# xvyaward/qeft

Measured on AMD Instinct MI355X. Metric: decode tokens/sec, Llama-2-7B w4 g128 r128, higher is better.
Workload: dtype f16; 1 GPU; llama-2-7b w4 g128 r128 full decode step, batch 1, greedy, KV context 69..1248 tokens (64-token context + 5 warm-up tokens before the timed region); layers=32, hipgraph=True, parallelism=single GPU

## Files before the change

include/qeft_hip.h:

```cpp
#ifndef QEFT_HIP_H
#define QEFT_HIP_H

#ifdef __cplusplus
extern "C" {
#endif

#define QEFT_OK 0
#define QEFT_ERR_BATCH 1
#define QEFT_ERR_SHAPE 2
#define QEFT_ERR_GROUP 3
#define QEFT_ERR_NULL 4
#define QEFT_ERR_LAUNCH 5
#define QEFT_ERR_ALIGN 6

typedef void* qeft_stream_t;

int qeft_abi_version(void);
const char* qeft_error_string(int code);
int qeft_last_hip_error(void);
const char* qeft_last_variant(void);

int qeft_gemv_w4(const void* x, const void* qweight, const void* scales, const void* scaled_zeros,
                 void* y, int m, int n, int k, int group_size, qeft_stream_t stream);

// ... 110 lines not shown
int qeft_token_begin_norm(const void* embed, const void* tok, const void* rope_tab, const int* pos, void* h32, void* rope_row,
                          const void* gamma, void* h_norm, float* ssq_out, int hidden, int vocab, int max_seq,
                          qeft_stream_t stream);
int qeft_rmsnorm_f32(const void* x32, const void* gamma, void* y, int m, int hidden, float eps, qeft_stream_t stream);
int qeft_rope_rows(void* x, const void* cos_tab, const void* sin_tab, int t, int n_heads, int row_stride,
                   qeft_stream_t stream);
int qeft_lm_head_f16(const void* h32, const void* gamma, const void* weight, void* logits, int hidden, int vocab, float eps,
                     qeft_stream_t stream);
int qeft_residual_norm(const void* h32, const void* add, const void* gamma, void* h32_out, void* h_norm, float* ssq_out,
                       int hidden, qeft_stream_t stream);

int qeft_gemm_w3_supported(int m, int n, int k, int group_size, int n_out);
int qeft_gemm_w3(const void* x, const void* qweight3, const void* scales, const void* scaled_zeros, const void* oweight,
                 const void* bias, void* y, int m, int n, int k, int group_size, int n_out, qeft_stream_t stream);
int qeft_gemm_w3_dx_supported(int m, int n, int k, int group_size, int n_out);
int qeft_gemm_w3_dx(const void* dy, const void* qweight3, const void* scales, const void* scaled_zeros, const void* oweight,
                    void* dx, int m, int n, int k, int group_size, int n_out, qeft_stream_t stream);

int qeft_gemv_w3(const void* x, const void* qweight3, const void* scales, const void* scaled_zeros,
                 const void* oweight_il, const void* bias, const void* residual, const void* sz_packed, void* y, int m,
                 int n, int k, int group_size, int n_out, qeft_stream_t stream);
int qeft_gemv_w3_group(const void* x, const void* norm_gamma, float norm_eps, int nparts,
                       const void* const* qweight3, const void* const* scales, const void* const* scaled_zeros,
                       const void* const* oweight_il, const void* const* bias, const void* const* sz_packed,
                       void* const* y, const int* n, int k, int group_size, int n_out, qeft_stream_t stream);
int qeft_gemv_w3_silu(const void* gate, const void* up, const void* qweight3, const void* scales,
                      const void* scaled_zeros, const void* oweight_il, const void* bias, const void* residual,
                      const void* sz_packed, void* y, int n, int k, int group_size, int n_out, qeft_stream_t stream);
int qeft_expand_w3(const void* qweight3, void* qweight4, int n, int k, int n_out, qeft_stream_t stream);

int qeft_token_begin(const void* embed, const void* tok, const void* rope_tab, const int* pos, void* h, void* rope_row,
                     int hidden, int vocab, int max_seq, qeft_stream_t stream);
int qeft_token_end(const void* logits, void* tok, int* pos, int vocab, int greedy, qeft_stream_t stream);

int qeft_decode_linear_m(const void* x, const void* qweight, const void* sz_packed, const void* oweight, const void* bias,
                         void* y, int n, int k, int group_size, int n_out, int mode, const void* residual,
                         const float* ssq_in, int n_ssq_in, float eps, const void* gamma_out, void* y_norm, float* ssq_out,
                         int m, qeft_stream_t stream);
long long qeft_gemv_v3_check_extents_m(int n, int k, int group_size, int n_out, int m, int mode, int n_ssq_in, int shrink_rows);
int qeft_token_begin_norm_m(const void* embed, const void* tokens, const void* rope_tab, const int* pos, void* h, void* rope_rows,
                            const void* gamma, void* h_norm, float* ssq_out, int hidden, int vocab, int max_seq, int m,
                            qeft_stream_t stream);
int qeft_attn_m_workspace_bytes(int n_heads, int n_split, int m);
int qeft_rope_attn_decode_m(const void* q, const void* k, const void* v, int qkv_stride, const void* cos_tab, const void* sin_tab,
                            int tab_stride, int tab_rows, void* k_cache, void* v_cache, const int* pos, const int* out_pos,
                            void* out, int out_stride, void* workspace, int n_split, int n_heads, int n_kv_heads, int max_seq,
                            int m, qeft_stream_t stream);
int qeft_lm_head_f16_m(const void* h32, const void* gamma, const void* weight, void* logits, int hidden, int vocab, float eps,
                       int m, qeft_stream_t stream);
int qeft_verify_greedy(const void* logits, const void* tokens, int m, int vocab, int greedy, void* out_tokens, int* n_accepted,
                       void* tok, int* pos, qeft_stream_t stream);

int qeft_token_begin_norm_batch(const void* embed, const void* tokens, const void* rope_tab, const int* slots, const int* pos, void* h,
                                void* rope_rows, const void* gamma, void* h_norm, float* ssq_out, int hidden, int vocab, int max_seq,
                                int n_slots, int m, qeft_stream_t stream);
int qeft_attn_batch_workspace_bytes(int n_heads, int n_split, int m);
int qeft_rope_attn_decode_batch(const void* q, const void* k, const void* v, int qkv_stride, const void* cos_tab, const void* sin_tab,
                                int tab_stride, int tab_rows, void* k_cache, void* v_cache, const int* slots, const int* pos,
                                const int* done, const int* out_pos, void* out, int out_stride, void* workspace, int n_split,
                                int n_slots, int n_heads, int n_kv_heads, int max_seq, int m, qeft_stream_t stream);
int qeft_token_end_batch(const void* logits, const int* slots, void* tokens, int* pos, const int* limit, const int* eos, int* done,
                         void* out, int* counter, int vocab, int out_cap, int n_slots, int m, qeft_stream_t stream);

int qeft_attn_kv8_workspace_bytes(int n_heads, int n_split, int m);
int qeft_rope_attn_decode_kv8(const void* q, const void* k, const void* v, int qkv_stride, const void* cos_tab, const void* sin_tab,
                              int tab_stride, int tab_rows, void* k_codes, void* v_codes, void* k_scales, void* v_scales,
// ... 107 lines not shown
```

qeft_amd/csrc/capi.hip:

```cpp
#include <hip/hip_runtime.h>

#include <cstdlib>
#include <cstring>
#include <stdint.h>

#include "../../include/qeft_hip.h"
#include "qeft_common.h"
#include "host_launch.h"
#include "gemm_w4.h"
#include "gemv_v3.h"
#include "decode_rows.h"
#include "decode_kv8.h"
#include "prefill_attn.h"
#include "attn_train.h"
#include "train_glue.h"

static thread_local int g_last_hip_error = 0;
thread_local const char* qeft::g_last_variant = "";
static bool small_m_route(int m, int n, bool have_workspace = false) {
    if (m <= 16) return true;
    if (have_workspace) return false;
    const int slices = (m + 15) / 16;
    return m <= 64 && (long long)slices * n <= 16384;
}
// ... 727 lines not shown
                          qeft_stream_t stream) {
    if (hidden < 8 || hidden % 8 != 0 || vocab < 1 || max_seq < 1) return QEFT_ERR_SHAPE;
    if (!embed || !tok || !h || !gamma || !h_norm || !ssq_out || (rope_row && (!rope_tab || !pos))) return QEFT_ERR_NULL;
    if (!aligned16(embed) || !aligned16(h) || !aligned16(gamma) || !aligned16(h_norm)) return QEFT_ERR_ALIGN;
    return finish(qeft::token_begin_norm_launch(embed, tok, rope_tab, pos, h, rope_row, gamma, h_norm, ssq_out, hidden, vocab,
                                                max_seq, (hipStream_t)stream));
}

int qeft_residual_norm(const void* h, const void* add, const void* gamma, void* h_out, void* h_norm, float* ssq_out,
                       int hidden, qeft_stream_t stream) {
    if (hidden < 8 || hidden % 8 != 0) return QEFT_ERR_SHAPE;
    if (!h || !h_out) return QEFT_ERR_NULL;
    if (gamma && (!h_norm || !ssq_out)) return QEFT_ERR_NULL;
    if (!aligned16(h) || !aligned16(h_out) || (add && !aligned16(add)) || (gamma && (!aligned16(gamma) || !aligned16(h_norm))))
        return QEFT_ERR_ALIGN;
    return finish(qeft::residual_norm_launch(h, add, gamma, h_out, h_norm, ssq_out, hidden, (hipStream_t)stream));
}

int qeft_token_begin(const void* embed, const void* tok, const void* rope_tab, const int* pos, void* h, void* rope_row,
                     int hidden, int vocab, int max_seq, qeft_stream_t stream) {
    if (hidden < 8 || hidden % 8 != 0 || vocab < 1 || max_seq < 1) return QEFT_ERR_SHAPE;
    if (!embed || !tok || !h || (rope_row && (!rope_tab || !pos))) return QEFT_ERR_NULL;
    if (!aligned16(embed) || !aligned16(h)) return QEFT_ERR_ALIGN;
    return finish(qeft::token_begin_launch(embed, tok, rope_tab, pos, h, rope_row, hidden, vocab, max_seq, (hipStream_t)stream));
}

int qeft_token_end(const void* logits, void* tok, int* pos, int vocab, int greedy, qeft_stream_t stream) {
    if (vocab < 1) return QEFT_ERR_SHAPE;
    if (!pos || (greedy && (!logits || !tok))) return QEFT_ERR_NULL;
    if (greedy && !aligned16(logits)) return QEFT_ERR_ALIGN;
    return finish(qeft::token_end_launch(logits, tok, pos, vocab, greedy, (hipStream_t)stream));
}

static bool verify_m_ok(int m) { return m >= 1 && m <= 8; }

int qeft_decode_linear_m(const void* x, const void* qweight, const void* sz_packed, const void* oweight, const void* bias,
                         void* y, int n, int k, int group_size, int n_out, int mode, const void* residual,
                         const float* ssq_in, int n_ssq_in, float eps, const void* gamma_out, void* y_norm, float* ssq_out,
                         int m, qeft_stream_t stream) {
    if (!verify_m_ok(m)) return QEFT_ERR_BATCH;
    if (m == 1)
        return qeft_decode_linear(x, qweight, sz_packed, oweight, bias, y, n, k, group_size, n_out, mode, residual, ssq_in, n_ssq_in,
                                  eps, gamma_out, y_norm, ssq_out, stream);
    if (int e = decode_linear_operands(x, qweight, 16, sz_packed, oweight, y, n_out)) return e;
    qeft::V3Args a;
    if (int e = v3_args(a, x, qweight, sz_packed, oweight, bias, y, n, k, group_size, n_out, mode)) return e;
    if (a.g.ngroups == 1 && k > 128) return QEFT_ERR_GROUP;
    if (int e = decode_linear_epilogue(a, mode, y, residual, ssq_in, n_ssq_in, eps, gamma_out, y_norm, ssq_out)) return e;
    a.m = m;
    hipError_t e = qeft::gemv_v3_multi_launch(a, mode, (hipStream_t)stream);
    if (e == hipErrorInvalidValue) return QEFT_ERR_SHAPE;
    return finish(e);
}

long long qeft_gemv_v3_check_extents_m(int n, int k, int group_size, int n_out, int m, int mode, int n_ssq_in, int shrink_rows) {
    qeft::V3Geom G{};
    if (!verify_m_ok(m) || v3_geom(G, n, k, group_size, n_out, mode) != QEFT_OK) return -1;
    if (G.ngroups == 1 && k > 128) return -1;
    if (n_ssq_in < 0 || n_ssq_in > qeft::V3_MAX_SSQ || shrink_rows < 0 || shrink_rows % 16 != 0 || shrink_rows >= n) return -1;
    return qeft::gemv_v3_count_out_of_range(G, n - shrink_rows, 0, false, 4) +
           qeft::gemv_v3_count_out_of_range_multi(G, n - shrink_rows, m, mode, n_ssq_in);
}

int qeft_token_begin_norm_m(const void* embed, const void* tokens, const void* rope_tab, const int* pos, void* h, void* rope_rows,
                            const void* gamma, void* h_norm, float* ssq_out, int hidden, int vocab, int max_seq, int m,
                            qeft_stream_t stream) {
// ... 597 lines not shown
```

qeft_amd/csrc/decode_aux.hip:

```cpp
#include <cstdlib>

#include "qeft_common.h"
#include "host_launch.h"
#include "decode_attn.h"

namespace qeft {

__device__ __forceinline__ float block_sum_256(float v, float* sm) {
    v = wave_sum(v);
    const int lane = threadIdx.x & 63, wave = threadIdx.x >> 6;
    __syncthreads();
    if (lane == 0) sm[wave] = v;
    __syncthreads();
    return sm[0] + sm[1] + sm[2] + sm[3];
}

__device__ __forceinline__ float block_max_256(float v, float* sm) {
#pragma unroll
    for (int o = 32; o > 0; o >>= 1) v = fmaxf(v, __shfl_xor(v, o));
    const int lane = threadIdx.x & 63, wave = threadIdx.x >> 6;
    __syncthreads();
    if (lane == 0) sm[wave] = v;
    __syncthreads();
    return fmaxf(fmaxf(sm[0], sm[1]), fmaxf(sm[2], sm[3]));
// ... 124 lines not shown
__global__ __launch_bounds__(256) void rmsnorm_f32_kernel(const float* __restrict__ x, const f16* __restrict__ gamma,
                                                          f16* __restrict__ y, int H, float eps) {
    __shared__ float sm[4];
    const size_t base = (size_t)blockIdx.x * H;
    float ss = 0.f;
    for (int i = threadIdx.x; i < H; i += 256) ss += x[base + i] * x[base + i];
    ss = block_sum_256(ss, sm);
    const float rs = rsqrtf(ss / (float)H + eps);
    for (int i = threadIdx.x; i < H; i += 256) y[base + i] = mul_f32_to_f16(x[base + i] * rs, (float)gamma[i]);
}

__global__ __launch_bounds__(256) void rope_rows_kernel(f16* __restrict__ x, const float* __restrict__ cs,
                                                        const float* __restrict__ sn, int H, int row_stride) {
    const int t = blockIdx.x, i = threadIdx.x & 63;
    const float c = cs[(size_t)t * 64 + i], s = sn[(size_t)t * 64 + i];
    for (int h = threadIdx.x >> 6; h < H; h += 4) {
        f16* p = x + (size_t)t * row_stride + h * 128;
        const float a = (float)p[i], b = (float)p[i + 64];
        p[i] = (f16)(a * c - b * s);
        p[i + 64] = (f16)(b * c + a * s);
    }
}

hipError_t rope_rows_launch(void* x, const void* cs, const void* sn, int T, int H, int row_stride, hipStream_t st) {
    hipLaunchKernelGGL(rope_rows_kernel, dim3(T), dim3(256), 0, st, (f16*)x, (const float*)cs, (const float*)sn, H, row_stride);
    return hipGetLastError();
}

template <int LPR>
__global__ __launch_bounds__(512) void lm_head_f16_kernel(const float* __restrict__ h32, const f16* __restrict__ gamma,
                                                          const f16* __restrict__ W, f16* __restrict__ logits, int vocab,
                                                          float eps, int rows_per_block) {
    constexpr int H = 512 * LPR;
    __shared__ float red[8];
    const int tid = threadIdx.x, lane = tid & 63;
    const int wave = __builtin_amdgcn_readfirstlane(tid >> 6);
    float xv[LPR][8];
    float ss = 0.f;
#pragma unroll
    for (int c = 0; c < LPR; ++c) {
        const f32x4 a = *(const f32x4*)(h32 + c * 512 + lane * 8), b = *(const f32x4*)(h32 + c * 512 + lane * 8 + 4);
#pragma unroll
        for (int j = 0; j < 4; ++j) {
            xv[c][j] = a[j];
            xv[c][4 + j] = b[j];
            ss += a[j] * a[j] + b[j] * b[j];
        }
    }
    ss = wave_sum(ss);
    const float rs = rsqrtf(ss / (float)H + eps);
    h2 xh[LPR][4];
#pragma unroll
    for (int c = 0; c < LPR; ++c) {
        const h8 g = *(const h8*)(gamma + c * 512 + lane * 8);
#pragma unroll
        for (int j = 0; j < 4; ++j)
            xh[c][j] = h2{mul_f32_to_f16(xv[c][2 * j] * rs, (float)g[2 * j]), mul_f32_to_f16(xv[c][2 * j + 1] * rs, (float)g[2 * j + 1])};
    }
    (void)red;
    const int r_end = min(vocab, (int)(blockIdx.x + 1) * rows_per_block);
    int r = blockIdx.x * rows_per_block + wave;
    u32x4 cur[LPR], nxt[LPR];
    auto load_row = [&](int row, u32x4 (&dst)[LPR]) {
        const u32x4* p = (const u32x4*)(W + (size_t)min(row, vocab - 1) * H) + lane;
#pragma unroll
        for (int c = 0; c < LPR; ++c) dst[c] = __builtin_nontemporal_load(p + c * 64);
    };
    load_row(r, cur);
    for (; r < r_end; r += 8) {
        load_row(r + 8, nxt);
        float acc = 0.f;
#pragma unroll
        for (int c = 0; c < LPR; ++c)
#pragma unroll
            for (int j = 0; j < 4; ++j) acc = __builtin_amdgcn_fdot2(as_h2(cur[c][j]), xh[c][j], acc, false);
        acc = wave_sum(acc);
        if (lane == 0) logits[r] = (f16)acc;
#pragma unroll
        for (int c = 0; c < LPR; ++c) cur[c] = nxt[c];
    }
}

hipError_t lm_head_f16_launch(const void* h32, const void* gamma, const void* W, void* logits, int H, int vocab, float eps,
                              hipStream_t st) {
    const int blocks = vocab >= 4096 ? 512 : (vocab + 7) / 8, rpb = (vocab + blocks - 1) / blocks;
    auto go = [&](auto kern) {
        hipLaunchKernelGGL(kern, dim3(blocks), dim3(512), 0, st, (const float*)h32, (const f16*)gamma, (const f16*)W, (f16*)logits,
                           vocab, eps, rpb);
        return hipGetLastError();
    };
    switch (H) {
        case 512: return go(lm_head_f16_kernel<1>);
        case 1024: return go(lm_head_f16_kernel<2>);
        case 2048: return go(lm_head_f16_kernel<4>);
        case 4096: return go(lm_head_f16_kernel<8>);
        case 5120: return go(lm_head_f16_kernel<10>);
        case 8192: return go(lm_head_f16_kernel<16>);
        default: return hipErrorInvalidValue;
    }
}

__global__ __launch_bounds__(1024) void token_end_kernel(const f16* __restrict__ logits, long long* __restrict__ tok,
                                                         int* __restrict__ pos, int vocab, int greedy) {
    __shared__ float bv[16];
    __shared__ int bi[16];
    const int t = threadIdx.x;
    if (greedy) {
        float best = -INFINITY;
        int idx = 0x7fffffff;
        for (int i = t * 8; i < vocab; i += 1024 * 8) {
            if (i + 8 <= vocab) {
                const h8 v = *(const h8*)(logits + i);
#pragma unroll
                for (int j = 0; j < 8; ++j)
                    if ((float)v[j] > best) { best = (float)v[j]; idx = i + j; }
            } else {
                for (int j = i; j < vocab; ++j)
                    if ((float)logits[j] > best) { best = (float)logits[j]; idx = j; }
            }
        }
#pragma unroll
        for (int o = 32; o > 0; o >>= 1) {
            const float ob = __shfl_xor(best, o);
            const int oi = __shfl_xor(idx, o);
            if (ob > best || (ob == best && oi < idx)) { best = ob; idx = oi; }
        }
        if ((t & 63) == 0) { bv[t >> 6] = best; bi[t >> 6] = idx; }
        __syncthreads();
        if (t == 0) {
            for (int w = 1; w < 16; ++w)
                if (bv[w] > best || (bv[w] == best && bi[w] < idx)) { best = bv[w]; idx = bi[w]; }
            *tok = idx == 0x7fffffff ? 0 : idx;
        }
    }
    if (t == 0) *pos = *pos + 1;
}

hipError_t token_begin_launch(const void* embed, const void* tok, const void* rope_tab, const int* pos, void* h,
                              void* rope_row, int hidden, int vocab, int max_seq, hipStream_t st) {
    hipLaunchKernelGGL(token_begin_kernel, dim3((hidden / 8 + 255) / 256), dim3(256), 0, st, (const f16*)embed,
                       (const long long*)tok, (const float*)rope_tab, pos, (f16*)h, (float*)rope_row, hidden, vocab, max_seq);
    return hipGetLastError();
}

int token_begin_norm_blocks(int hidden) { return (hidden / 8 + 255) / 256; }

hipError_t token_begin_norm_launch(const void* embed, const void* tok, const void* rope_tab, const int* pos, void* h,
                                   void* rope_row, const void* gamma, void* hnorm, float* ssq_out, int hidden, int vocab,
                                   int max_seq, hipStream_t st) {
    hipLaunchKernelGGL(token_begin_norm_kernel, dim3(token_begin_norm_blocks(hidden)), dim3(256), 0, st, (const f16*)embed,
                       (const long long*)tok, (const float*)rope_tab, pos, (float*)h, (float*)rope_row, (const f16*)gamma,
                       (f16*)hnorm, ssq_out, hidden, vocab, max_seq);
    return hipGetLastError();
}

hipError_t residual_norm_launch(const void* h, const void* add, const void* gamma, void* h_out, void* hnorm, float* ssq_out,
                                int hidden, hipStream_t st) {
    hipLaunchKernelGGL(residual_norm_kernel, dim3(token_begin_norm_blocks(hidden)), dim3(256), 0, st, (const float*)h,
                       (const f16*)add, (const f16*)gamma, (float*)h_out, (f16*)hnorm, ssq_out, hidden);
    return hipGetLastError();
}

hipError_t rmsnorm_f32_launch(const void* x, const void* gamma, void* y, int m, int H, float eps, hipStream_t st) {
    hipLaunchKernelGGL(rmsnorm_f32_kernel, dim3(m), dim3(256), 0, st, (const float*)x, (const f16*)gamma, (f16*)y, H, eps);
    return hipGetLastError();
}

hipError_t token_end_launch(const void* logits, void* tok, int* pos, int vocab, int greedy, hipStream_t st) {
    hipLaunchKernelGGL(token_end_kernel, dim3(1), dim3(1024), 0, st, (const f16*)logits, (long long*)tok, pos, vocab, greedy);
    return hipGetLastError();
}

hipError_t rmsnorm_launch(const void* x, const void* add, const void* gamma, void* res_out, void* y, int m, int H,
                          float eps, hipStream_t st) {
    hipLaunchKernelGGL(rmsnorm_kernel, dim3(m), dim3(256), 0, st, (const f16*)x, (const f16*)add, (const f16*)gamma,
                       (f16*)res_out, (f16*)y, H, eps);
    return hipGetLastError();
}

hipError_t silu_mul_launch(const void* gate, const void* up, void* out, int n, hipStream_t st) {
    hipLaunchKernelGGL(silu_mul_kernel, dim3((n / 8 + 255) / 256), dim3(256), 0, st, (const f16*)gate, (const f16*)up,
                       (f16*)out, n);
    return hipGetLastError();
}

unsigned long long* g_attn_dbg = nullptr;
#ifndef QEFT_ATTN_PRE1
#define QEFT_ATTN_PRE1 4
#endif
size_t attn_workspace_bytes(int n_heads, int S) { return S > 1 ? (attn_ctr_floats(n_heads) + (size_t)n_heads * S * kAttnRec) * 4 : 0; }

hipError_t rope_attn_decode_launch(const void* q, const void* k, const void* v, const void* cs, const void* sn, void* kc,
                                   void* vc, const int* pos, const int* out_pos, void* out, void* ws, int n_heads,
                                   int n_kv, int max_seq, int S, int tab_rows, hipStream_t st, bool k_ft_layout,
                                   const float* alibi_slopes) {
    const size_t smem = (size_t)(max_seq + 16) * 4 + 16 * 128 * 4 + 64 * 4 + 4 * 4 + 3 * 128 * 2;
    int dh = 1;
    auto launch = [&](auto kern) -> hipError_t {
        if (smem > 64 * 1024) {
            hipError_t e = hipFuncSetAttribute((const void*)kern, hipFuncAttributeMaxDynamicSharedMemorySize, (int)smem);
            if (e != hipSuccess) return e;
        }
// ... 133 lines not shown
```

qeft_amd/csrc/decode_verify.hip:

```cpp
#include "qeft_common.h"
#include "decode_attn.h"
#include "decode_rows.h"
#include "host_launch.h"

namespace qeft {

typedef float fx2 __attribute__((ext_vector_type(2)));

__global__ __launch_bounds__(256) void token_begin_norm_m_kernel(const f16* __restrict__ embed, const long long* __restrict__ toks,
                                                                 const float* __restrict__ rope_tab, const int* __restrict__ pos,
                                                                 float* __restrict__ h, float* __restrict__ rope_rows,
                                                                 const f16* __restrict__ gamma, f16* __restrict__ hnorm,
                                                                 float* __restrict__ ssq_out, int hidden, int vocab, int max_seq) {
    token_begin_norm_row(embed, toks, rope_tab, h, rope_rows, gamma, hnorm, ssq_out, hidden, vocab, max_seq,
                         [&](int row) { return *pos + row; });
}

hipError_t token_begin_norm_m_launch(const void* embed, const void* toks, const void* rope_tab, const int* pos, void* h,
                                     void* rope_rows, const void* gamma, void* hnorm, float* ssq_out, int hidden, int vocab,
                                     int max_seq, int m, hipStream_t st) {
    hipLaunchKernelGGL(token_begin_norm_m_kernel, dim3(token_begin_norm_blocks(hidden), m), dim3(256), 0, st, (const f16*)embed,
                       (const long long*)toks, (const float*)rope_tab, pos, (float*)h, (float*)rope_rows, (const f16*)gamma,
                       (f16*)hnorm, ssq_out, hidden, vocab, max_seq);
    return hipGetLastError();
// ... 248 lines not shown

size_t attn_m_workspace_bytes(int n_heads, int S, int m) { return S > 1 ? (attn_m_ctr_floats(n_heads) + (size_t)n_heads * m * S * kAttnRec) * 4 : 0; }

hipError_t rope_attn_m_launch(const AttnRowsArgs& a, hipStream_t st) {
    const int grp = a.n_heads / a.n_kv, hc = attn_m_chunk(grp, a.m), rows = hc * a.m;
    const int R = rows <= 8 ? 8 : rows <= 16 ? 16 : 32;
    const size_t smem = attn_m_smem_bytes(R);
    auto go = [&](auto kern) -> hipError_t {
        if (smem > 64 * 1024) {
            hipError_t e = hipFuncSetAttribute((const void*)kern, hipFuncAttributeMaxDynamicSharedMemorySize, (int)smem);
            if (e != hipSuccess) return e;
        }
        hipLaunchKernelGGL(kern, dim3(a.n_kv * (grp / hc) * a.S), dim3(256), smem, st, a.pos, a.out_pos, (const f16*)a.q, (const f16*)a.k,
                           (const f16*)a.v, (const float*)a.cs, (const float*)a.sn, (f16*)a.kc, (f16*)a.vc, (f16*)a.out, (float*)a.ws,
                           a.qkv_stride, a.out_stride, a.tab_stride, a.tab_rows, a.max_seq, a.n_heads, a.n_kv, a.S, a.m, hc);
        return hipGetLastError();
    };
    if (R == 8) return go(rope_attn_m_kernel<8>);
    if (R == 16) return go(rope_attn_m_kernel<16>);
    return go(rope_attn_m_kernel<32>);
}

template <int LPR>
__global__ __launch_bounds__(512) void lm_head_m_kernel(const float* __restrict__ h32, const f16* __restrict__ gamma,
                                                        const f16* __restrict__ W, f16* __restrict__ logits, int vocab, float eps,
                                                        int rows_per_block, int m) {
    constexpr int H = 512 * LPR;
    extern __shared__ __attribute__((aligned(16))) uint8_t smem_raw[];
    h8* const xs = (h8*)smem_raw;
    const int tid = threadIdx.x, lane = tid & 63;
    const int wave = __builtin_amdgcn_readfirstlane(tid >> 6);
    if (wave < m) {
        const float* hr = h32 + (size_t)wave * H;
        float xv[LPR][8];
        float ss = 0.f;
#pragma unroll
        for (int c = 0; c < LPR; ++c) {
            const f32x4 a = *(const f32x4*)(hr + c * 512 + lane * 8), b = *(const f32x4*)(hr + c * 512 + lane * 8 + 4);
#pragma unroll
            for (int j = 0; j < 4; ++j) {
                xv[c][j] = a[j];
                xv[c][4 + j] = b[j];
                ss += a[j] * a[j] + b[j] * b[j];
            }
        }
        ss = wave_sum(ss);
        const float rs = rsqrtf(ss / (float)H + eps);
#pragma unroll
        for (int c = 0; c < LPR; ++c) {
            const h8 g = *(const h8*)(gamma + c * 512 + lane * 8);
            h8 o;
#pragma unroll
            for (int j = 0; j < 8; ++j) o[j] = mul_f32_to_f16(xv[c][j] * rs, (float)g[j]);
            xs[((size_t)wave * LPR + c) * 64 + lane] = o;
        }
    }
    __syncthreads();
    const int r_end = min(vocab, (int)(blockIdx.x + 1) * rows_per_block);
    int r = blockIdx.x * rows_per_block + wave;
    u32x4 cur[LPR], nxt[LPR];
    auto load_row = [&](int row, u32x4 (&dst)[LPR]) {
        const u32x4* p = (const u32x4*)(W + (size_t)min(row, vocab - 1) * H) + lane;
#pragma unroll
        for (int c = 0; c < LPR; ++c) dst[c] = __builtin_nontemporal_load(p + c * 64);
    };
    load_row(r, cur);
    for (; r < r_end; r += 8) {
        load_row(r + 8, nxt);
        for (int i = 0; i < m; ++i) {
            float acc = 0.f;
#pragma unroll
            for (int c = 0; c < LPR; ++c) {
                const u32x4 xw = __builtin_bit_cast(u32x4, xs[((size_t)i * LPR + c) * 64 + lane]);
#pragma unroll
                for (int j = 0; j < 4; ++j) acc = __builtin_amdgcn_fdot2(as_h2(cur[c][j]), as_h2(xw[j]), acc, false);
            }
            acc = wave_sum(acc);
            if (lane == 0) logits[(size_t)i * vocab + r] = (f16)acc;
        }
#pragma unroll
        for (int c = 0; c < LPR; ++c) cur[c] = nxt[c];
    }
}

hipError_t lm_head_m_launch(const void* h32, const void* gamma, const void* W, void* logits, int H, int vocab, float eps, int m,
                            hipStream_t st) {
// ... 60 lines not shown
```

qeft_amd/csrc/host_launch.h:

```cpp
#pragma once
#include "qeft_common.h"

namespace qeft {

hipError_t token_begin_launch(const void* embed, const void* tok, const void* rope_tab, const int* pos, void* h,
                              void* rope_row, int hidden, int vocab, int max_seq, hipStream_t st);
int token_begin_norm_blocks(int hidden);
hipError_t token_begin_norm_launch(const void* embed, const void* tok, const void* rope_tab, const int* pos, void* h,
                                   void* rope_row, const void* gamma, void* hnorm, float* ssq_out, int hidden, int vocab,
                                   int max_seq, hipStream_t st);
hipError_t token_end_launch(const void* logits, void* tok, int* pos, int vocab, int greedy, hipStream_t st);
hipError_t residual_norm_launch(const void* h, const void* add, const void* gamma, void* h_out, void* hnorm, float* ssq_out,
                                int hidden, hipStream_t st);
hipError_t rmsnorm_launch(const void* x, const void* add, const void* gamma, void* res_out, void* y, int m, int H,
                          float eps, hipStream_t st);
hipError_t rmsnorm_f32_launch(const void* x, const void* gamma, void* y, int m, int H, float eps, hipStream_t st);
hipError_t rope_rows_launch(void* x, const void* cs, const void* sn, int T, int H, int row_stride, hipStream_t st);
hipError_t silu_mul_launch(const void* gate, const void* up, void* out, int n, hipStream_t st);
hipError_t lm_head_f16_launch(const void* h32, const void* gamma, const void* W, void* logits, int H, int vocab, float eps,
                              hipStream_t st);
size_t attn_workspace_bytes(int n_heads, int S);
hipError_t rope_attn_decode_launch(const void* q, const void* k, const void* v, const void* cs, const void* sn, void* kc,
                                   void* vc, const int* pos, const int* out_pos, void* out, void* ws, int n_heads,
                                   int n_kv, int max_seq, int S, int tab_rows, hipStream_t st, bool k_ft_layout = false,
                                   const float* alibi_slopes = nullptr);
hipError_t sqa_generic_launch(const void* q, const void* k, const void* v, void* kc, void* vc, const int* pos, const float* alibi,
                              void* out, int n_heads, int n_kv, int max_seq, int head_dim, hipStream_t st);
extern unsigned long long* g_attn_dbg;

hipError_t sample_launch(const void* logits, int vocab, int m, const int* params, const int* positions, void* tokens,
                         hipStream_t st);
hipError_t token_end_sample_launch(const void* logits, void* tok, int* pos, const int* params, int vocab, hipStream_t st);
hipError_t verify_sample_launch(const void* logits, const void* tokens, int m, int vocab, const int* params, int* work, void* out_tokens,
                                int* n_acc, void* tok, int* pos, hipStream_t st);
hipError_t token_end_sample_b_launch(const void* logits, const int* slot_tab, void* tok, int* pos_tab, const int* limit, const int* eos,
                                     int* done, void* out, int* ctr, const int* params, int vocab, int out_cap, int n_slots, int m,
                                     hipStream_t st);

hipError_t gemv_w4_dispatch(const GemvArgs& a, int m, hipStream_t st);
hipError_t gemv_w4_group_dispatch(GemvGroupArgs g, int nparts, hipStream_t st);
hipError_t gemv_w4_silu_dispatch(const GemvArgs& a, hipStream_t st);
hipError_t gemv_w4_smallm_dispatch(const GemvArgs& a, int m, hipStream_t st);
hipError_t gemv_w3_dispatch(const GemvArgs& a, int m, hipStream_t st);
hipError_t gemv_w3_group_dispatch(GemvGroupArgs g, int nparts, hipStream_t st);
// ... 24 lines not shown
```

qeft_amd/llama.py:

```python
import ctypes
import os
import math
import types
from dataclasses import dataclass

import torch
import torch.nn as nn

from . import _lib, fuse, qeft_cuda
from .qlinear import QuantLinear
from .quant import fake_quantize, minmax_params


@dataclass
class LlamaShape:
    hidden: int
    inter: int
    n_layers: int
    n_heads: int
    n_kv_heads: int
    vocab: int
    max_seq: int = 512
    rms_eps: float = 1e-5
    rope_theta: float = 10000.0
# ... 910 lines not shown
        self._head(h32, self.hn, self.logits, None, st)
        self._token_end(st)

    def _lin_m(self, b, m, st):
        s, lib = self.m.shape, self.lib
        g, no, eps = s.group_size, s.n_out, s.rms_eps
        xn, ssq = b.xn.data_ptr(), b.ssq.data_ptr()

        def lin(op, x, y, mode=0, residual=None, ssq_in=None, n_ssq=0, gamma_out=None):
            return lib.qeft_decode_linear_m(x, op.qweight.data_ptr(), op.sz_packed.data_ptr(), op.oweight.data_ptr() if no else None,
                                            None, y, op.outfeatures, op.infeatures, g, no, mode, residual, ssq_in, n_ssq, eps,
                                            gamma_out, xn if gamma_out else None, ssq if gamma_out else None, m, st)
        return lin

    def _v3_layers(self, b, lin, attn, only=None):
        ck, layers = _lib.check, self.m.model.layers
        xn, ssq, h32 = b.xn.data_ptr(), b.ssq.data_ptr(), b.h32.data_ptr()
        qkv, att, act = b.qkv.data_ptr(), b.att.data_ptr(), b.act.data_ptr()

        lin_qkv, lin_o, lin_gu, lin_d = (lin if only in (None, tag) else (lambda *a, **kw: 0) for tag in ("qkv", "o", "gu", "d"))
        n_ssq = self.n_ssq_tb
        for li, L in enumerate(layers):
            pk = self.v3ops[li]
            ck(lin_qkv(pk["qkv"], xn, qkv, ssq_in=ssq, n_ssq=n_ssq))
            if attn is not None:
                attn(li)
            ck(lin_o(pk["o"], att, h32, residual=h32, gamma_out=L.post_attention_layernorm.weight.data_ptr()))
            n_ssq = self.n_ssq_lin
            ck(lin_gu(pk["gu"], xn, act, mode=1, ssq_in=ssq, n_ssq=n_ssq))
            nxt = layers[li + 1].input_layernorm.weight.data_ptr() if li + 1 < len(layers) else None
            ck(lin_d(pk["d"], act, h32, residual=h32, gamma_out=nxt))

    @torch.no_grad()
    def _launch_token_v3(self, linears_only=False, only=None):
        s, lib, ck, b = self.m.shape, self.lib, _lib.check, self.row1
        st = torch.cuda.current_stream(self.dev).cuda_stream
        g, no, eps = s.group_size, s.n_out, s.rms_eps
        xn, ssq, h32 = b.xn.data_ptr(), b.ssq.data_ptr(), b.h32.data_ptr()
        entry = lib.qeft_decode_linear_w3 if self.bits == 3 else lib.qeft_decode_linear

        def lin(op, x, y, mode=0, residual=None, ssq_in=None, n_ssq=0, gamma_out=None):
            return entry(x, op.qweight.data_ptr(), op.sz_packed.data_ptr(), op.oweight.data_ptr() if no else None, None, y,
                         op.outfeatures, op.infeatures, g, no, mode, residual, ssq_in, n_ssq, eps, gamma_out,
                         xn if gamma_out else None, ssq if gamma_out else None, st)
        if linears_only:
            return self._v3_layers(b, lin, None, only)
        ck(lib.qeft_token_begin_norm(self.m.model.embed_tokens.weight.data_ptr(), self.tok.data_ptr(), self.rope_tab.data_ptr(),
                                     self.pos.data_ptr(), h32, self.rope_row.data_ptr(),
                                     self.m.model.layers[0].input_layernorm.weight.data_ptr(), xn, ssq, s.hidden, s.vocab,
                                     s.max_seq, st))
        q, k, v = self.q.data_ptr(), self.k.data_ptr(), self.v.data_ptr()
        self._v3_layers(b, lin, lambda li: self._attn(li, q, k, v, self.att_pos[li], self.att, st), only)
        self._token_tail(h32, st)

    @torch.no_grad()
    def _launch_token_tp3(self, linears_only=False, only=None):
        s, lib, ck = self.m.shape, self.lib, _lib.check
        st = torch.cuda.current_stream(self.dev).cuda_stream
        g, no, eps = s.group_size, s.n_out, s.rms_eps
        layers = self.m.model.layers
        cur, oth = self.h32, self.part32
        zero = self.zero32.data_ptr()

        def hnorm(op, h, gamma, y, mode=0):
            return lib.qeft_decode_linear_hnorm(h.data_ptr(), gamma.data_ptr(), op.qweight.data_ptr(), op.sz_packed.data_ptr(),
                                                op.oweight.data_ptr() if no else None, None, y, op.outfeatures, op.infeatures, g,
                                                no, mode, eps, st)

        def partial(op, x, h, y):
            return lib.qeft_decode_linear(x, op.qweight.data_ptr(), op.sz_packed.data_ptr(), op.oweight.data_ptr() if no else None,
                                          None, y.data_ptr(), op.outfeatures, op.infeatures, g, no, 0,
                                          h.data_ptr() if self.rank == 0 else zero, None, 0, eps, None, None, None, st)

        def pick(tag, fn):
            return fn if only in (None, tag) else (lambda *a, **kw: 0)
        if not linears_only:
            ck(lib.qeft_token_begin_norm(self.m.model.embed_tokens.weight.data_ptr(), self.tok.data_ptr(),
                                         self.rope_tab.data_ptr(), self.pos.data_ptr(), cur.data_ptr(), self.rope_row.data_ptr(),
                                         layers[0].input_layernorm.weight.data_ptr(), self.xn.data_ptr(), self.ssq.data_ptr(), s.hidden,
                                         s.vocab, s.max_seq, st))
        qp = self.qkv_loc.data_ptr()
        for li, L in enumerate(layers):
            pk = self.tp3ops[li]
            ck(pick("qkv", hnorm)(pk["qkv"], cur, L.input_layernorm.weight, qp))
            if not linears_only:
                self._attn(li, qp, qp + self.hs * 2, qp + (self.hs + self.kvs) * 2, pk["att_pos"], pk["x_o"], st)
# ... 46 lines not shown
        self.sample_rec.copy_(torch.tensor(params.record(), dtype=torch.int32))
        self.sampling = params

    def step(self):
        if self.host_pos >= self.m.shape.max_seq:
            raise RuntimeError(f"KV cache full: position {self.host_pos} >= max_seq {self.m.shape.max_seq}")
        self._check_fresh()
        sp = self._split_for(self.host_pos)
        if self.use_graph:
            g = self.graphs.get(self._step_key(sp))
            if g is None:
                g = self.capture(split=sp)
            g.replay()
        else:
            self.attn_split = sp
            self._launch_token()
        self.host_pos += 1

    MULTI = int(os.environ.get("QEFT_MULTI_TOKENS", "8"))

    def run(self, n_tokens):
        assert self.greedy or self.sampling is not None, \
            "run() feeds every token's successor to the next: greedy or sampled decoding only"
        self._check_fresh()
        multi_ok = self.use_graph and os.environ.get("QEFT_MULTI_TOKEN_GRAPH") != "0"
        while n_tokens > 0:
            p, m = self.host_pos, self.MULTI
            sp = self._split_for(p)
            if multi_ok and n_tokens >= m and p + m <= self.m.shape.max_seq and self._split_for(p + m - 1) == sp:
                key = (sp, "sample", m) if self.sampling is not None else (sp, True, m)
                g = self.graphs.get(key)
                if g is None:
                    self.attn_split = sp
                    g = self.graphs[key] = capture_graph(self.dev, self._launch_token, m, (self.pos, self.tok))
                g.replay()
                self.host_pos += m
                n_tokens -= m
            else:
                self.step()
                n_tokens -= 1

    VERIFY_MAX = 8

    def _m_row_unsupported(self):
        if self.tp or self.tp3:
            return "the verify pass runs on the single-GPU engine only (this engine is tensor-parallel)"
        if self.bits != 4:
            return f"the verify pass runs on 4-bit weights only (this engine has {self.bits}-bit weights)"
        if not self.v3:
            return "the verify pass runs on the v3 engine only (QEFT_ENGINE_V2=1, or shapes the v3 GEMV does not take)"
        return None

    def _verify_unsupported(self):
        why = self._m_row_unsupported()
        if why is None and self.kv_dtype != "fp16" and not getattr(self, "kv8_verify", False):
            return (f'the verify pass runs on an fp16 KV cache only (this engine has kv_dtype="{self.kv_dtype}"; '
                    f'build it with kv8_verify=True for the verify pass over an fp8 KV cache)')
        return why

    def _verify_bufs(self):
        vb = getattr(self, "_vb", None)
        if vb is not None:
            return vb
        s, dev, M = self.m.shape, self.dev, self.VERIFY_MAX
        ws_bytes = self.lib.qeft_attn_m_kv8_workspace_bytes if self.kv_dtype == "fp8" else self.lib.qeft_attn_m_workspace_bytes
        vb = m_row_buffers(self, M, ws_bytes(s.n_heads, 8, M))
        vb.toks = torch.zeros(M, dtype=torch.long, device=dev)
# ... 96 lines not shown
```

Measured before the change: 756.7 tokens/s.

## Fuse greedy argmax with next token's embed/norm/rope into one turn kernel

```diff
diff --git a/include/qeft_hip.h b/include/qeft_hip.h
--- a/include/qeft_hip.h
+++ b/include/qeft_hip.h
@@ -166,6 +166,8 @@
 int qeft_token_begin(const void* embed, const void* tok, const void* rope_tab, const int* pos, void* h, void* rope_row,
                      int hidden, int vocab, int max_seq, qeft_stream_t stream);
 int qeft_token_end(const void* logits, void* tok, int* pos, int vocab, int greedy, qeft_stream_t stream);
+int qeft_token_turn(const void* logits, void* tok, int* pos, const void* embed, const void* rope_tab, void* h32, void* rope_row,
+                    const void* gamma, void* h_norm, float* ssq_out, int hidden, int vocab, int max_seq, qeft_stream_t stream);
 
 int qeft_decode_linear_m(const void* x, const void* qweight, const void* sz_packed, const void* oweight, const void* bias,
                          void* y, int n, int k, int group_size, int n_out, int mode, const void* residual,
diff --git a/qeft_amd/csrc/capi.hip b/qeft_amd/csrc/capi.hip
--- a/qeft_amd/csrc/capi.hip
+++ b/qeft_amd/csrc/capi.hip
@@ -783,6 +783,15 @@
     return finish(qeft::token_end_launch(logits, tok, pos, vocab, greedy, (hipStream_t)stream));
 }
 
+int qeft_token_turn(const void* logits, void* tok, int* pos, const void* embed, const void* rope_tab, void* h, void* rope_row,
+                    const void* gamma, void* h_norm, float* ssq_out, int hidden, int vocab, int max_seq, qeft_stream_t stream) {
+    if (hidden < 8 || hidden % 8 != 0 || hidden > 8192 || vocab < 1 || max_seq < 1) return QEFT_ERR_SHAPE;
+    if (!logits || !tok || !pos || !embed || !rope_tab || !h || !rope_row || !gamma || !h_norm || !ssq_out) return QEFT_ERR_NULL;
+    if (!aligned16(logits) || !aligned16(embed) || !aligned16(h) || !aligned16(gamma) || !aligned16(h_norm)) return QEFT_ERR_ALIGN;
+    return finish(qeft::token_turn_launch(logits, tok, pos, embed, rope_tab, h, rope_row, gamma, h_norm, ssq_out, hidden, vocab,
+                                          max_seq, (hipStream_t)stream));
+}
+
 static bool verify_m_ok(int m) { return m >= 1 && m <= 8; }
 
 int qeft_decode_linear_m(const void* x, const void* qweight, const void* sz_packed, const void* oweight, const void* bias,
diff --git a/qeft_amd/csrc/decode_aux.hip b/qeft_amd/csrc/decode_aux.hip
--- a/qeft_amd/csrc/decode_aux.hip
+++ b/qeft_amd/csrc/decode_aux.hip
@@ -180,43 +180,56 @@
                                                           const f16* __restrict__ W, f16* __restrict__ logits, int vocab,
                                                           float eps, int rows_per_block) {
     constexpr int H = 512 * LPR;
-    __shared__ float red[8];
+    constexpr int CUR0 = LPR == 16 ? 0 : LPR == 8 ? 4 : LPR;
+    constexpr int XH0 = LPR == 8 ? 2 : LPR;
     const int tid = threadIdx.x, lane = tid & 63;
     const int wave = __builtin_amdgcn_readfirstlane(tid >> 6);
-    float xv[LPR][8];
+    const int r_end = min(vocab, (int)(blockIdx.x + 1) * rows_per_block);
+    int r = blockIdx.x * rows_per_block + wave;
+    if (r >= r_end) return;
+    u32x4 cur[LPR], nxt[LPR];
+    auto load_row = [&](int row, u32x4 (&dst)[LPR], int c0, int c1) {
+        const u32x4* p = (const u32x4*)(W + (size_t)min(row, vocab - 1) * H) + lane;
+#pragma unroll
+        for (int c = c0; c < c1; ++c) dst[c] = __builtin_nontemporal_load(p + c * 64);
+    };
+    f32x4 xa[LPR], xb[LPR];
+    h8 g[LPR];
+#pragma unroll
+    for (int c = 0; c < LPR; ++c) {
+        xa[c] = *(const f32x4*)(h32 + c * 512 + lane * 8);
+        xb[c] = *(const f32x4*)(h32 + c * 512 + lane * 8 + 4);
+    }
+#pragma unroll
+    for (int c = 0; c < LPR; ++c) g[c] = *(const h8*)(gamma + c * 512 + lane * 8);
+    load_row(r, cur, 0, CUR0);
+    __builtin_amdgcn_sched_barrier(0);
     float ss = 0.f;
 #pragma unroll
-    for (int c = 0; c < LPR; ++c) {
-        const f32x4 a = *(const f32x4*)(h32 + c * 512 + lane * 8), b = *(const f32x4*)(h32 + c * 512 + lane * 8 + 4);
-#pragma unroll
-        for (int j = 0; j < 4; ++j) {
-            xv[c][j] = a[j];
-            xv[c][4 + j] = b[j];
-            ss += a[j] * a[j] + b[j] * b[j];
-        }
-    }
+    for (int c = 0; c < LPR; ++c)
+#pragma unroll
+        for (int j = 0; j < 4; ++j) ss += xa[c][j] * xa[c][j] + xb[c][j] * xb[c][j];
     ss = wave_sum(ss);
     const float rs = rsqrtf(ss / (float)H + eps);
     h2 xh[LPR][4];
-#pragma unroll
-    for (int c = 0; c < LPR; ++c) {
-        const h8 g = *(const h8*)(gamma + c * 512 + lane * 8);
-#pragma unroll
-        for (int j = 0; j < 4; ++j)
-            xh[c][j] = h2{mul_f32_to_f16(xv[c][2 * j] * rs, (float)g[2 * j]), mul_f32_to_f16(xv[c][2 * j + 1] * rs, (float)g[2 * j + 1])};
-    }
-    (void)red;
-    const int r_end = min(vocab, (int)(blockIdx.x + 1) * rows_per_block);
-    int r = blockIdx.x * rows_per_block + wave;
-    u32x4 cur[LPR], nxt[LPR];
-    auto load_row = [&](int row, u32x4 (&dst)[LPR]) {
-        const u32x4* p = (const u32x4*)(W + (size_t)min(row, vocab - 1) * H) + lane;
-#pragma unroll
-        for (int c = 0; c < LPR; ++c) dst[c] = __builtin_nontemporal_load(p + c * 64);
+    auto norm_chunk = [&](int c) {
+#pragma unroll
+        for (int j = 0; j < 2; ++j) {
+            xh[c][j] = h2{mul_f32_to_f16(xa[c][2 * j] * rs, (float)g[c][2 * j]), mul_f32_to_f16(xa[c][2 * j + 1] * rs, (float)g[c][2 * j + 1])};
+            xh[c][2 + j] = h2{mul_f32_to_f16(xb[c][2 * j] * rs, (float)g[c][4 + 2 * j]), mul_f32_to_f16(xb[c][2 * j + 1] * rs, (float)g[c][4 + 2 * j + 1])};
+        }
     };
-    load_row(r, cur);
-    for (; r < r_end; r += 8) {
-        load_row(r + 8, nxt);
+#pragma unroll
+    for (int c = 0; c < XH0; ++c) norm_chunk(c);
+    if constexpr (CUR0 < LPR) {
+        __builtin_amdgcn_sched_barrier(0);
+        load_row(r, cur, CUR0, LPR);
+        __builtin_amdgcn_sched_barrier(0);
+    }
+#pragma unroll
+    for (int c = XH0; c < LPR; ++c) norm_chunk(c);
+    do {
+        load_row(r + 8, nxt, 0, LPR);
         float acc = 0.f;
 #pragma unroll
         for (int c = 0; c < LPR; ++c)
@@ -226,7 +239,8 @@
         if (lane == 0) logits[r] = (f16)acc;
 #pragma unroll
         for (int c = 0; c < LPR; ++c) cur[c] = nxt[c];
-    }
+        r += 8;
+    } while (r < r_end);
 }
 
 hipError_t lm_head_f16_launch(const void* h32, const void* gamma, const void* W, void* logits, int H, int vocab, float eps,
@@ -248,40 +262,116 @@
     }
 }
 
+__device__ __forceinline__ int greedy_argmax_1024(const f16* __restrict__ logits, int vocab, float* bv, int* bi) {
+    constexpr int kPass = 1024 * 8, kPre = 4;
+    const int t = threadIdx.x;
+    float best = -INFINITY;
+    int idx = 0x7fffffff;
+    auto tail = [&](int i) {
+        for (int j = i; j < vocab; ++j)
+            if ((float)logits[j] > best) { best = (float)logits[j]; idx = j; }
+    };
+    if (vocab <= kPre * kPass) {
+        h8 v[kPre] = {};
+        if (vocab >= 8) {
+            const int last = (vocab & ~7) - 8;
+#pragma unroll
+            for (int p = 0; p < kPre; ++p) v[p] = *(const h8*)(logits + min(t * 8 + p * kPass, last));
+        }
+        __builtin_amdgcn_sched_barrier(0);
+#pragma unroll
+        for (int p = 0; p < kPre; ++p) {
+            const int i = t * 8 + p * kPass;
+            if (i + 8 <= vocab) {
+#pragma unroll
+                for (int j = 0; j < 8; ++j)
+                    if ((float)v[p][j] > best) { best = (float)v[p][j]; idx = i + j; }
+            } else if (i < vocab) {
+                tail(i);
+            }
+        }
+    } else {
+        for (int i = t * 8; i < vocab; i += kPass) {
+            if (i + 8 <= vocab) {
+                const h8 v = *(const h8*)(logits + i);
+#pragma unroll
+                for (int j = 0; j < 8; ++j)
+                    if ((float)v[j] > best) { best = (float)v[j]; idx = i + j; }
+            } else {
+                tail(i);
+            }
+        }
+    }
+#pragma unroll
+    for (int o = 32; o > 0; o >>= 1) {
+        const float ob = __shfl_xor(best, o);
+        const int oi = __shfl_xor(idx, o);
+        if (ob > best || (ob == best && oi < idx)) { best = ob; idx = oi; }
+    }
+    if ((t & 63) == 0) { bv[t >> 6] = best; bi[t >> 6] = idx; }
+    __syncthreads();
+    if (t == 0)
+        for (int w = 1; w < 16; ++w)
+            if (bv[w] > best || (bv[w] == best && bi[w] < idx)) { best = bv[w]; idx = bi[w]; }
+    return idx == 0x7fffffff ? 0 : idx;
+}
+
 __global__ __launch_bounds__(1024) void token_end_kernel(const f16* __restrict__ logits, long long* __restrict__ tok,
                                                          int* __restrict__ pos, int vocab, int greedy) {
     __shared__ float bv[16];
     __shared__ int bi[16];
     const int t = threadIdx.x;
     if (greedy) {
-        float best = -INFINITY;
-        int idx = 0x7fffffff;
-        for (int i = t * 8; i < vocab; i += 1024 * 8) {
-            if (i + 8 <= vocab) {
-                const h8 v = *(const h8*)(logits + i);
-#pragma unroll
-                for (int j = 0; j < 8; ++j)
-                    if ((float)v[j] > best) { best = (float)v[j]; idx = i + j; }
-            } else {
-                for (int j = i; j < vocab; ++j)
-                    if ((float)logits[j] > best) { best = (float)logits[j]; idx = j; }
-            }
-        }
-#pragma unroll
-        for (int o = 32; o > 0; o >>= 1) {
-            const float ob = __shfl_xor(best, o);
-            const int oi = __shfl_xor(idx, o);
-            if (ob > best || (ob == best && oi < idx)) { best = ob; idx = oi; }
-        }
-        if ((t & 63) == 0) { bv[t >> 6] = best; bi[t >> 6] = idx; }
-        __syncthreads();
-        if (t == 0) {
-            for (int w = 1; w < 16; ++w)
-                if (bv[w] > best || (bv[w] == best && bi[w] < idx)) { best = bv[w]; idx = bi[w]; }
-            *tok = idx == 0x7fffffff ? 0 : idx;
-        }
+        const int idx = greedy_argmax_1024(logits, vocab, bv, bi);
+        if (t == 0) *tok = idx;
     }
     if (t == 0) *pos = *pos + 1;
+}
+
+__global__ __launch_bounds__(1024) void token_turn_kernel(const f16* __restrict__ logits, long long* __restrict__ tok,
+                                                          int* __restrict__ pos, const f16* __restrict__ embed,
+                                                          const float* __restrict__ rope_tab, float* __restrict__ h,
+                                                          float* __restrict__ rope_row, const f16* __restrict__ gamma,
+                                                          f16* __restrict__ hnorm, float* __restrict__ ssq_out, int hidden,
+                                                          int vocab, int max_seq) {
+    __shared__ float bv[16];
+    __shared__ int bi[16];
+    __shared__ float sm[16];
+    __shared__ int tok_s;
+    const int t = threadIdx.x, i = t * 8;
+    const int p1 = *pos + 1;
+    const bool mine = i < hidden, rope = t >= 896 && rope_row;
+    const h8 g = *(const h8*)(gamma + (mine ? i : 0));
+    const float rv = rope_tab[(size_t)min(max(p1, 0), max_seq - 1) * 128 + (rope ? t - 896 : 0)];
+    __builtin_amdgcn_sched_barrier(0);
+    const int idx = greedy_argmax_1024(logits, vocab, bv, bi);
+    if (t == 0) {
+        *tok = idx;
+        *pos = p1;
+        tok_s = idx;
+    }
+    __syncthreads();
+    const int tk = min(max(tok_s, 0), vocab - 1);
+    float ss = 0.f;
+    if (mine) {
+        const h8 v = *(const h8*)(embed + (size_t)tk * hidden + i);
+        h8 o;
+#pragma unroll
+        for (int j = 0; j < 8; ++j) {
+            ss += (float)v[j] * (float)v[j];
+            o[j] = mul_f32_to_f16((float)v[j], (float)g[j]);
+            h[i + j] = (float)v[j];
+        }
+        *(h8*)(hnorm + i) = o;
+    }
+    ss = wave_sum(ss);
+    if ((t & 63) == 0) sm[t >> 6] = ss;
+    __syncthreads();
+    if ((t & 255) == 0 && t * 8 < hidden) {
+        const int w = t >> 6;
+        ssq_out[t >> 8] = sm[w] + sm[w + 1] + sm[w + 2] + sm[w + 3];
+    }
+    if (rope) rope_row[t - 896] = rv;
 }
 
 hipError_t token_begin_launch(const void* embed, const void* tok, const void* rope_tab, const int* pos, void* h,
@@ -316,6 +406,15 @@
 
 hipError_t token_end_launch(const void* logits, void* tok, int* pos, int vocab, int greedy, hipStream_t st) {
     hipLaunchKernelGGL(token_end_kernel, dim3(1), dim3(1024), 0, st, (const f16*)logits, (long long*)tok, pos, vocab, greedy);
+    return hipGetLastError();
+}
+
+hipError_t token_turn_launch(const void* logits, void* tok, int* pos, const void* embed, const void* rope_tab, void* h,
+                             void* rope_row, const void* gamma, void* hnorm, float* ssq_out, int hidden, int vocab, int max_seq,
+                             hipStream_t st) {
+    hipLaunchKernelGGL(token_turn_kernel, dim3(1), dim3(1024), 0, st, (const f16*)logits, (long long*)tok, pos, (const f16*)embed,
+                       (const float*)rope_tab, (float*)h, (float*)rope_row, (const f16*)gamma, (f16*)hnorm, ssq_out, hidden, vocab,
+                       max_seq);
     return hipGetLastError();
 }
 
diff --git a/qeft_amd/csrc/decode_verify.hip b/qeft_amd/csrc/decode_verify.hip
--- a/qeft_amd/csrc/decode_verify.hip
+++ b/qeft_amd/csrc/decode_verify.hip
@@ -304,26 +304,31 @@
     const int wave = __builtin_amdgcn_readfirstlane(tid >> 6);
     if (wave < m) {
         const float* hr = h32 + (size_t)wave * H;
-        float xv[LPR][8];
+        f32x4 xa[LPR], xb[LPR];
+        h8 g[LPR];
+#pragma unroll
+        for (int c = 0; c < LPR; ++c) {
+            xa[c] = *(const f32x4*)(hr + c * 512 + lane * 8);
+            xb[c] = *(const f32x4*)(hr + c * 512 + lane * 8 + 4);
+        }
+#pragma unroll
+        for (int c = 0; c < LPR; ++c) g[c] = *(const h8*)(gamma + c * 512 + lane * 8);
+        __builtin_amdgcn_sched_barrier(0);
         float ss = 0.f;
 #pragma unroll
-        for (int c = 0; c < LPR; ++c) {
-            const f32x4 a = *(const f32x4*)(hr + c * 512 + lane * 8), b = *(const f32x4*)(hr + c * 512 + lane * 8 + 4);
-#pragma unroll
-            for (int j = 0; j < 4; ++j) {
-                xv[c][j] = a[j];
-                xv[c][4 + j] = b[j];
-                ss += a[j] * a[j] + b[j] * b[j];
-            }
-        }
+        for (int c = 0; c < LPR; ++c)
+#pragma unroll
+            for (int j = 0; j < 4; ++j) ss += xa[c][j] * xa[c][j] + xb[c][j] * xb[c][j];
         ss = wave_sum(ss);
         const float rs = rsqrtf(ss / (float)H + eps);
 #pragma unroll
         for (int c = 0; c < LPR; ++c) {
-            const h8 g = *(const h8*)(gamma + c * 512 + lane * 8);
             h8 o;
 #pragma unroll
-            for (int j = 0; j < 8; ++j) o[j] = mul_f32_to_f16(xv[c][j] * rs, (float)g[j]);
+            for (int j = 0; j < 4; ++j) {
+                o[j] = mul_f32_to_f16(xa[c][j] * rs, (float)g[c][j]);
+                o[4 + j] = mul_f32_to_f16(xb[c][j] * rs, (float)g[c][4 + j]);
+            }
             xs[((size_t)wave * LPR + c) * 64 + lane] = o;
         }
     }
diff --git a/qeft_amd/csrc/host_launch.h b/qeft_amd/csrc/host_launch.h
--- a/qeft_amd/csrc/host_launch.h
+++ b/qeft_amd/csrc/host_launch.h
@@ -10,6 +10,9 @@
                                    void* rope_row, const void* gamma, void* hnorm, float* ssq_out, int hidden, int vocab,
                                    int max_seq, hipStream_t st);
 hipError_t token_end_launch(const void* logits, void* tok, int* pos, int vocab, int greedy, hipStream_t st);
+hipError_t token_turn_launch(const void* logits, void* tok, int* pos, const void* embed, const void* rope_tab, void* h,
+                             void* rope_row, const void* gamma, void* hnorm, float* ssq_out, int hidden, int vocab, int max_seq,
+                             hipStream_t st);
 hipError_t residual_norm_launch(const void* h, const void* add, const void* gamma, void* h_out, void* hnorm, float* ssq_out,
                                 int hidden, hipStream_t st);
 hipError_t rmsnorm_launch(const void* x, const void* add, const void* gamma, void* res_out, void* y, int m, int H,
diff --git a/qeft_amd/llama.py b/qeft_amd/llama.py
--- a/qeft_amd/llama.py
+++ b/qeft_amd/llama.py
@@ -966,7 +966,7 @@
             ck(lin_d(pk["d"], act, h32, residual=h32, gamma_out=nxt))
 
     @torch.no_grad()
-    def _launch_token_v3(self, linears_only=False, only=None):
+    def _launch_token_v3(self, linears_only=False, only=None, begin=True, turn=False):
         s, lib, ck, b = self.m.shape, self.lib, _lib.check, self.row1
         st = torch.cuda.current_stream(self.dev).cuda_stream
         g, no, eps = s.group_size, s.n_out, s.rms_eps
@@ -979,13 +979,26 @@
                          xn if gamma_out else None, ssq if gamma_out else None, st)
         if linears_only:
             return self._v3_layers(b, lin, None, only)
-        ck(lib.qeft_token_begin_norm(self.m.model.embed_tokens.weight.data_ptr(), self.tok.data_ptr(), self.rope_tab.data_ptr(),
-                                     self.pos.data_ptr(), h32, self.rope_row.data_ptr(),
-                                     self.m.model.layers[0].input_layernorm.weight.data_ptr(), xn, ssq, s.hidden, s.vocab,
-                                     s.max_seq, st))
+        embed, gamma0 = self.m.model.embed_tokens.weight.data_ptr(), self.m.model.layers[0].input_layernorm.weight.data_ptr()
+        if begin:
+            ck(lib.qeft_token_begin_norm(embed, self.tok.data_ptr(), self.rope_tab.data_ptr(), self.pos.data_ptr(), h32,
+                                         self.rope_row.data_ptr(), gamma0, xn, ssq, s.hidden, s.vocab, s.max_seq, st))
         q, k, v = self.q.data_ptr(), self.k.data_ptr(), self.v.data_ptr()
         self._v3_layers(b, lin, lambda li: self._attn(li, q, k, v, self.att_pos[li], self.att, st), only)
-        self._token_tail(h32, st)
+        if not turn:
+            return self._token_tail(h32, st)
+        self._head(h32, self.hn, self.logits, None, st)
+        ck(lib.qeft_token_turn(self.logits.data_ptr(), self.tok.data_ptr(), self.pos.data_ptr(), embed, self.rope_tab.data_ptr(),
+                               h32, self.rope_row.data_ptr(), gamma0, xn, ssq, s.hidden, s.vocab, s.max_seq, st))
+
+    def _turn_ok(self):
+        return (self.v3 and self.greedy and self.sampling is None and self.m.shape.hidden <= 8192
+                and os.environ.get("QEFT_TOKEN_TURN") != "0")
+
+    def _launch_tokens_turn(self, m):
+        self.n_collectives = 0
+        for i in range(m):
+            self._launch_token_v3(begin=i == 0, turn=i < m - 1)
 
     @torch.no_grad()
     def _launch_token_tp3(self, linears_only=False, only=None):
@@ -1098,7 +1111,11 @@
                 g = self.graphs.get(key)
                 if g is None:
                     self.attn_split = sp
-                    g = self.graphs[key] = capture_graph(self.dev, self._launch_token, m, (self.pos, self.tok))
+                    if self._turn_ok():
+                        g = capture_graph(self.dev, lambda: self._launch_tokens_turn(m), 1, (self.pos, self.tok))
+                    else:
+                        g = capture_graph(self.dev, self._launch_token, m, (self.pos, self.tok))
+                    self.graphs[key] = g
                 g.replay()
                 self.host_pos += m
                 n_tokens -= m
```

New measurement: 753.1 tokens/s. No clear change (-0.5%).
